# Pyrokine/LineSegmentDetector-SLAM

Hardware: AMD Instinct MI355X
Metric: Mpixels/sec LSD (grad+grow+NFA) (higher is better)
Workload: dtype f64; 1 GPU; 512 x 2048x2048 u8 occupancy maps per GPU tiled/rolled/flipped from 4 aisle-class fixtures (SURVEY 8d C4), full pipeline incl. lineIm, params 0.3/0.6/22.5/0.7/1024; images_total=512, images_rank0=512, parallelism=single GPU, rccl_gather_in_step=False, steps_in_flight=8, steps_in_flight_asked=8, region_waves_per_image=4, help_across_workgroups=False, last_steps_with_help=0, writeback_map=False

## Files before the change

include/lsd_hip.h:

```cpp
#ifndef LSD_HIP_H
#define LSD_HIP_H
#include <stddef.h>
#include <stdint.h>

#ifdef __cplusplus
extern "C" {
#endif

#define LSD_ABI_VERSION 1

enum {
    LSD_OK = 0,
    LSD_ERR_INVALID = 1,
    LSD_ERR_NO_DEVICE = 2,
    LSD_ERR_HIP = 3,
    LSD_ERR_UNSUPPORTED = 4,
    LSD_ERR_CAPACITY = 5,
    LSD_ERR_NOMEM = 6,
    LSD_ERR_INTERNAL = 7
};

typedef struct lsd_params {
    double sca;
    double sig;
// ... 213 lines not shown
                      lsd_grid_match_rec *out, lsd_grid_match_mr_stats *stats);

void lsd_scaled_size(int cols, int rows, double sca, int *w, int *h);

enum { LSD_STAGE_ALL = 0, LSD_STAGE_GAUSS = 1, LSD_STAGE_GRAD = 2, LSD_STAGE_SORT = 3, LSD_STAGE_REGION = 4 };
int lsd_set_stop_after(lsd_ctx *ctx, int stage);
int lsd_set_trace(lsd_ctx *ctx, int on);
int lsd_set_fused_front(lsd_ctx *ctx, int on);
int lsd_set_region_waves(lsd_ctx *ctx, int waves);
int lsd_set_region_help(lsd_ctx *ctx, int waves);
int lsd_set_cost_history(lsd_ctx *ctx, int on);
int lsd_debug_set_stamp_budget(lsd_ctx *ctx, unsigned grows);
int lsd_debug_set_tuning(lsd_ctx *ctx, const char *name, int value);

enum { LSD_DBG_GAUSS = 1, LSD_DBG_MAG, LSD_DBG_DEG, LSD_DBG_STATE, LSD_DBG_ORDER, LSD_DBG_ORDER_VAL,
       LSD_DBG_NB, LSD_DBG_MAXGRAD, LSD_DBG_RECS, LSD_DBG_SEEDS, LSD_DBG_NSEED, LSD_DBG_STATS };
int lsd_debug_fetch(lsd_ctx *ctx, int image, int what, void *out, size_t bytes);

int lsd_debug_eval_math(lsd_ctx *ctx, int fn, const double *a, const double *b, double *out0, double *out1, size_t n);

int lsd_debug_lines(lsd_ctx *ctx, const double *recs, int n, int cols, int rows, lsd_line *lines_out, uint8_t *line_im);

int lsd_debug_calibrate(lsd_ctx *ctx, size_t bytes);

int lsd_last_timings(lsd_ctx *ctx, float ms_out[6]);

#ifdef __cplusplus
}
#endif
#endif
```

linesegmentdetector-slam_amd/__init__.py:

```python
import ctypes as C
import os

import numpy as np

_HERE = os.path.dirname(os.path.abspath(__file__))
LIB_PATH = os.path.join(_HERE, "liblsdhip.so")

LSD_OK, LSD_ERR_INVALID, LSD_ERR_NO_DEVICE, LSD_ERR_HIP, LSD_ERR_UNSUPPORTED, LSD_ERR_CAPACITY, LSD_ERR_NOMEM, LSD_ERR_INTERNAL = range(8)
LSD_FLAG_WRITEBACK_MAP = 1
STAGE_ALL, STAGE_GAUSS, STAGE_GRAD, STAGE_SORT, STAGE_REGION = range(5)
(DBG_GAUSS, DBG_MAG, DBG_DEG, DBG_STATE, DBG_ORDER, DBG_ORDER_VAL, DBG_NB, DBG_MAXGRAD, DBG_RECS, DBG_SEEDS,
 DBG_NSEED, DBG_STATS) = range(1, 13)

lsd_sca, lsd_sig, lsd_angThre, lsd_denThre, pseBin = 0.3, 0.6, 22.5, 0.7, 1024
z_occ_max_dis = 1.0
HOST_MAX_LINES_DEFAULT = 8192
rdp_leastPoint, rdp_threLine, rdp_leastDist = 3, 0.08, 0.5


class lsd_params(C.Structure):
    _fields_ = [("sca", C.c_double), ("sig", C.c_double), ("angThre", C.c_double), ("denThre", C.c_double),
                ("pseBin", C.c_int)]


class lsd_line(C.Structure):
    _fields_ = [(n, C.c_double) for n in ("k", "b", "dx", "dy", "x1", "y1", "x2", "y2", "len")] + [("orient", C.c_int)]

# ... 664 lines not shown
            d = dict(zip(("grow_calls", "grown_px", "nfa_calls", "rrr_calls", "rrr_passes", "rrr_sentinel_drops",
                          "rrr_oob_reads", "cycles_refill", "cycles_total", "cycles_grow", "cycles_rect",
                          "cycles_nfa", "cycles_mark", "small_bails", "wait_noslot", "seeds", "exact_angle_evals",
                          "tile_fetches", "batches", "cycles_tiles", "spec_redos", "spec_discards", "cycles_wait", "small_steps",
                          "refill_rounds", "cycles_eval", "cycles_sums", "cycles_refine", "cycles_small", "cycles_select", "cycles_commit",
                          "wait_noseed", "requeued_ahead", "cycles_eval_at_cursor", "depth_end", "nfa_min_abs_enc", "nfa_min_gap_enc", "help_exports", "help_evals", "near_ties",
                          "wd_commit", "wd_next", "wd_nseeds", "wd_state", "wd_nbig", "wd_lock", "wd_pend", "wd_wave"),
                         [int(x) for x in v]))
            d["set_answers"], d["sets_founded"] = int(v[41]), int(v[42])
            d["cycles_nfa_count"], d["nfa_tail_iters"] = int(v[43]), int(v[44])
            d["nfa_bracket_misses"] = int(v[40])
            for k in ("nfa_min_abs", "nfa_min_gap"):
                enc = d.pop(k + "_enc")
                d[k] = float("inf") if enc == 0 else float(np.array([0x7ff0000000000000 - enc], np.uint64).view(np.float64)[0])
            return d
        if what == DBG_SEEDS:
            ns = self.fetch(image, DBG_NSEED, shape_wh)
            return get(what, SEED_DTYPE, ns)
        raise ValueError(what)

    def eval_math(self, fn, a, b=None):
        a = np.ascontiguousarray(a, np.float64)
        b = None if b is None else np.ascontiguousarray(b, np.float64)
        o0, o1 = np.zeros_like(a), np.zeros_like(a)
        self._chk(self.L.lsd_debug_eval_math(self.h, fn, a.ctypes.data, None if b is None else b.ctypes.data,
                                             o0.ctypes.data, o1.ctypes.data, a.size))
        return o0, o1

    def debug_lines(self, recs, rows, cols, want_lineim=True):
        r = np.ascontiguousarray(recs, np.float64).reshape(-1, 4)
# ... 1036 lines not shown
```

linesegmentdetector-slam_amd/csrc/k_front.hip:

```cpp
#include "lsd_internal.h"
#include "k_front_lds.h"
#include "k1_stage.h"
#include "grad_px.h"

namespace lsdhip {

constexpr int TW = kK1TileW, TH = kK1TileH, NT = 256;
constexpr int GW = kFrontGW, GH = kFrontGH;
constexpr int HS = 17, TAPR = 8;
constexpr int PPT = TW * TH / NT;
static_assert(TW == 32 && TW * TH % NT == 0, "a thread keeps its column and walks down the tile NT / TW rows at a time");

__global__ __launch_bounds__(NT, 4) void k_front(const uint8_t* __restrict__ in, double* __restrict__ mag, double* __restrict__ deg,
                                                 double2* __restrict__ sc, uint32_t* __restrict__ pw, unsigned long long* __restrict__ maxbits,
                                                 int32_t* __restrict__ ties, const double* __restrict__ taps_g, const int* __restrict__ centre_of,
                                                 int W, int H, int w, int h, double gradThre, int IWp, unsigned strip_bytes, unsigned gx,
                                                 unsigned gy, unsigned tiles, uint8_t* __restrict__ clr) {
    extern __shared__ __align__(16) unsigned char smem[];
    double* aux = reinterpret_cast<double*>(smem);
    double* taps = reinterpret_cast<double*>(smem + strip_bytes);
    uint8_t* tile = reinterpret_cast<uint8_t*>(taps + 3 * HS);
    double* Gt = reinterpret_cast<double*>(tile);
    int* l_cnt = reinterpret_cast<int*>(Gt + GW * GH);
    unsigned long long* l_max = reinterpret_cast<unsigned long long*>(l_cnt + 2);
    double2* l_g = reinterpret_cast<double2*>(smem);
    uint32_t* l_px = reinterpret_cast<uint32_t*>(l_g + kFrontList);

    const int tid = threadIdx.x;
    const unsigned per = (tiles + 7u) >> 3;
    const unsigned t = (blockIdx.x & 7u) * per + (blockIdx.x >> 3);
    if (t >= tiles) return;
    const unsigned bx = t % gx, tq = t / gx, by = tq % gy;
// ... 13 lines not shown
    }
    const int Xf = max(X0 - 1, 0), Yf = max(Y0 - 1, 0);
    const int Xl = min(X0 + TW - 1, w - 1), Yl = min(Y0 + TH - 1, h - 1);
    const int c0 = centre_of[Xf] - TAPR, c1 = centre_of[Xl] + TAPR;
    const int r0 = centre_of[Yf] - TAPR, r1 = centre_of[Yl] + TAPR;
    const int IH = r1 - r0 + 1;

    for (int i = tid; i < 3 * HS; i += NT) taps[i] = taps_g[i];

    const int a0 = c0 - (((c0 % 4) + 4) % 4);
    const uint32_t wany = stage_window(src, tile, W, H, r0, r1, a0, c1, IWp, tid, 0u);

    const int X = tid & (TW - 1), Yt = tid / TW;
    const int gX = X0 + X;
    if (!__syncthreads_or((int)(wany != 0u))) {
        if (gX < w) {
            #pragma unroll
            for (int k = 0; k < PPT; k++) {
                const int gY = Y0 + Yt + k * (NT / TW);
                if (gY >= h) break;
                const GradPx px = grad_pixel(0.0, 0.0, 0.0, 0.0, gX >= 1 && gY >= 1, gradThre);
                const size_t p = base + (size_t)gY * w + gX;
                mag[p] = px.m;
                if (!px.heavy && px.u == 0) sc[p] = make_double2(0.0, 1.0);
                deg[p] = px.d;
                pw[p] = pack_pw(px.d, px.u);
            }
        }
        return;
    }
// ... 75 lines not shown
    }
    {
        unsigned long long bits = (unsigned long long)__double_as_longlong(mx);
        for (int off = 32; off >= 1; off >>= 1) {
            const unsigned long long o = __shfl_xor(bits, off);
            bits = o > bits ? o : bits;
        }
        if (lane == 0) l_max[wave] = bits;
    }
    __syncthreads();
    if (tid == 0) {
        unsigned long long bits = l_max[0];
        #pragma unroll
        for (int i = 1; i < NT / 64; i++) bits = l_max[i] > bits ? l_max[i] : bits;
        if (bits != 0ull) atomicMax(&maxbits[img], bits);
    }

    const int cnt = *l_cnt;
    for (int i = tid; i < cnt; i += NT) {
        const uint32_t e = l_px[i];
        const double2 gr = l_g[i];
        const double d = grad_angle(gr.x, gr.y, &ties[img]);
        l_g[i] = make_double2(d, 0.0);
        if (e & 1u) {
            const int lt = (int)(e >> 1);
            sc[base + (size_t)(Y0 + lt / TW) * w + (X0 + lt % TW)] = grad_sincos(d);
        }
    }
    __syncthreads();

// ... 9 lines not shown
            }
        }
    }
}

bool front_fits(const Geom& g, size_t max_lds) {
    if (2 * g.tapR + 1 != HS) return false;
    const size_t need = k_front_lds(g.sca, g.tapR).bytes;
    return need <= 64 * 1024 && need <= max_lds;
}

void launch_front(const Geom& g, const Buffers& b, int n, uint8_t* clr, hipStream_t s) {
    const KFrontLds L = k_front_lds(g.sca, g.tapR);
    const unsigned gx = (g.w + TW - 1) / TW, gy = (g.h + TH - 1) / TH, tiles = gx * gy * (unsigned)n;
    hipLaunchKernelGGL(k_front, dim3(((tiles + 7u) >> 3) * 8u), dim3(NT), L.bytes, s, b.in, b.mag, b.deg, b.sc, b.pw, b.maxbits, b.ties, b.taps,
                       b.centres, g.W, g.H, g.w, g.h, g.gradThre, L.IWp, (unsigned)L.strip, gx, gy, tiles, clr);
}

}
```

linesegmentdetector-slam_amd/csrc/k_sort.hip:

```cpp
#include "lsd_internal.h"

namespace lsdhip {

constexpr int SNT = 1024, SWAVES = SNT / 64;

__device__ __forceinline__ int bin_of(double m, double zoom, int pseBin) {
    int v = cvt_x86(floor(m * zoom));
    if (v > pseBin) v = pseBin;
    return (int)(uint16_t)v;
}

__global__ __launch_bounds__(SNT) void k_sort(const double* __restrict__ mag,
                                              const unsigned long long* __restrict__ maxbits,
                                              uint32_t* __restrict__ ord,
                                              int32_t* __restrict__ nb, uint32_t* __restrict__ kept_px, uint32_t* __restrict__ kept_v32,
                                              int npx, int pseBin) {
    extern __shared__ uint32_t hist[];
    uint32_t* wsum = hist + SWAVES * pseBin;
    const size_t img = blockIdx.x;
    const double* m = mag + img * (size_t)npx;
    uint32_t* o = ord + img * (size_t)npx;
    uint32_t* kp = kept_px + img * (size_t)npx;
    uint16_t* kv = reinterpret_cast<uint16_t*>(kept_v32 + img * (size_t)npx);
    const int tid = threadIdx.x, wave = tid >> 6, lane = tid & 63;

    const double maxGrad = __longlong_as_double((long long)maxbits[img]);
    if (!(maxGrad > 0)) {
        if (tid == 0) nb[img] = 0;
        return;
    }
    const double zoom = 1.0 * pseBin / maxGrad;
    const int segLen = ((npx + SNT - 1) / SNT) * 64;
    const int beg = min(wave * segLen, npx), end = min(beg + segLen, npx);

    for (int i = tid; i < SWAVES * pseBin; i += SNT) hist[i] = 0;
    __syncthreads();

    uint32_t* myh = hist + wave * pseBin;
    const unsigned long long lt = (1ull << lane) - 1ull;
    constexpr int UN = 4;
    int cnt = 0;
    for (int base = beg; base < end; base += 64 * UN) {
        double mv[UN];
        #pragma unroll
        for (int j = 0; j < UN; j++) {
            const int p = base + 64 * j + lane;
            mv[j] = p < end ? m[p] : 0.0;
        }
        #pragma unroll
        for (int j = 0; j < UN; j++) {
            const int v = bin_of(mv[j], zoom, pseBin);
            const unsigned long long km = __ballot(v != 0);
            if (v != 0) {
                atomicAdd(&myh[pseBin - v], 1u);
                const int k2 = beg + cnt + __builtin_popcountll(km & lt);
                kp[k2] = (uint32_t)(base + 64 * j + lane);
                kv[k2] = (uint16_t)v;
            }
            cnt += __builtin_popcountll(km);
        }
    }
    __syncthreads();

    {
        uint32_t tot = 0;
        if (tid < pseBin)
            for (int s = 0; s < SWAVES; s++) tot += hist[s * pseBin + tid];
        uint32_t inc = tot;
        for (int off = 1; off < 64; off <<= 1) {
            uint32_t t = __shfl_up(inc, off);
            if (lane >= off) inc += t;
        }
        if (lane == 63) wsum[wave] = inc;
        __syncthreads();
// ... 29 lines not shown
            for (int bit = 0; bit < nbits; bit++) {
                const bool one = ((b >> bit) & 1) != 0;
                const unsigned long long mk = __ballot(one);
                peers &= one ? mk : ~mk;
            }
            const uint32_t start = myh[b];
            if (act) {
                const uint32_t r = start + (uint32_t)__builtin_popcountll(peers & lt);
                o[r] = pv[j];
                if (((peers >> lane) >> 1) == 0ull) myh[b] = start + (uint32_t)__builtin_popcountll(peers);
            }
        }
    }
}

__global__ __launch_bounds__(256) void k_order(const int32_t* __restrict__ nb, const long long* __restrict__ hist, uint32_t* __restrict__ order, int n, int npx) {
    __shared__ uint32_t cnt[256];
    __shared__ uint32_t start[256];
    __shared__ unsigned long long hmax;
    const int tid = threadIdx.x;
    cnt[tid] = 0;
    if (tid == 0) hmax = 1ull;
    __syncthreads();
    if (hist) {
        unsigned long long m = 0;
        for (int i = tid; i < n; i += 256) m = max(m, (unsigned long long)max(hist[(size_t)i * kStatWords + kStatTotalWord], 0ll));
        atomicMax(&hmax, m);
        __syncthreads();
    }
    const unsigned long long hm = hmax;
    auto key = [&](int i) {
        if (hist) return 255 - (int)(((unsigned long long)max(hist[(size_t)i * kStatWords + kStatTotalWord], 0ll) * 255ull) / hm);
        return 255 - (int)min(255ll, (long long)nb[i] * 2048 / (npx + 1));
    };
    for (int i = tid; i < n; i += 256) atomicAdd(&cnt[key(i)], 1u);
    __syncthreads();
    if (tid == 0) {
        uint32_t run = 0;
        for (int k2 = 0; k2 < 256; k2++) { start[k2] = run; run += cnt[k2]; }
    }
    __syncthreads();
    uint32_t pos = start[tid];
    for (int i = 0; i < n; i++)
        if (key(i) == tid) order[pos++] = (uint32_t)i;
}

void launch_order(const Buffers& b, int n, int npx, const long long* hist, hipStream_t s) {
    hipLaunchKernelGGL(k_order, dim3(1), dim3(256), 0, s, b.nb, hist, b.order, n, npx);
}

__global__ __launch_bounds__(256) void k_ordv(const double* __restrict__ mag, const unsigned long long* __restrict__ maxbits, const uint32_t* __restrict__ ord,
                                              uint16_t* __restrict__ out, int count, int pseBin) {
    const int i = blockIdx.x * 256 + threadIdx.x;
    const double maxGrad = __longlong_as_double((long long)maxbits[0]);
    if (i < count && maxGrad > 0) out[i] = (uint16_t)bin_of(mag[ord[i]], 1.0 * pseBin / maxGrad, pseBin);
}
void launch_ordv(const double* mag, const unsigned long long* maxbits, const uint32_t* ord, uint16_t* out, int count, int pseBin, hipStream_t s) {
    if (count > 0) hipLaunchKernelGGL(k_ordv, dim3((count + 255) / 256), dim3(256), 0, s, mag, maxbits, ord, out, count, pseBin);
}

void launch_sort(const Geom& g, const Buffers& b, int n, hipStream_t s) {
    const size_t lds = ((size_t)SWAVES * g.pseBin + SWAVES) * sizeof(uint32_t);
    (void)hipFuncSetAttribute(reinterpret_cast<const void*>(k_sort), hipFuncAttributeMaxDynamicSharedMemorySize,
                              (int)lds);
    hipLaunchKernelGGL(k_sort, dim3(n), dim3(SNT), lds, s, b.mag, b.maxbits, b.ord, b.nb, b.seedidx, b.seedpos, g.npx, g.pseBin);
}

}
```

linesegmentdetector-slam_amd/csrc/lsd_ctx.hip:

```cpp
#include <math.h>
#include <stddef.h>
#include <stdio.h>
#include <stdlib.h>
#include <string.h>

#include <algorithm>
#include <mutex>
#include <string>
#include <vector>

#include "lsd_devbuf.h"
#include "lsd_internal.h"
#include "k1_lds.h"
#include "k_rdp_lds.h"

using namespace lsdhip;

struct Workspace {
    size_t cap_gpx = 0;
    size_t cap_n = 0, cap_npx = 0, cap_ws = 0;
    int cap_max_lines = 0;
    DevBuf<double> gauss, mag, deg, recs, recs_scaled;
    DevBuf<double2> sc;
    DevBuf<uint32_t> order;
    DevBuf<uint32_t> sets;
    DevBuf<uint32_t> pw, epochmap, ord, spill, gcopy, stamps, seedidx, seedpos, tepoch;
    uint32_t run_id = 0;
    DevBuf<uint32_t> slist;
    DevBuf<double> pend;
    DevBuf<float4> wmeta;
    DevBuf<int> rnum;
    DevBuf<uint32_t> xq;
    DevBuf<unsigned long long> maxbits;
    DevBuf<int32_t> nb, nseed;
    DevBuf<long long> stats;
    DevBuf<SeedRec> seeds;
    int32_t* ties() const { return reinterpret_cast<int32_t*>(maxbits.get() + cap_n); }
};

struct lsd_ctx {
    int device = 0;
    int num_cus = 256;
    size_t max_lds = 0;
    uint32_t id_budget = 0xFFFF0u;
    int tun_soft = 0, tun_claim = 0, tun_feed = 3, tun_big = 0;
    int tun_help = -1;
    int tun_gate = 12000;
    int tun_share = 0;
    int pool_max_images = 4;
    int tun_early = 0, tun_wb = 10, tun_up = 32, tun_down = 96, tun_requeue = 1, tun_xpoll = 20000, tun_linger = 1000000, tun_stop = 0;
    int region_waves_mode = 0;
    bool prefer4 = false;
// ... 39 lines not shown
    hipEvent_t ga_ev = nullptr;
    bool ga_ev_valid = false;
    int stop_after = 0;
    int tun_groups = -1;
    DevBuf<int> pcount;
    bool trace = false;
    bool fused_front = true;
    int scan_cap = kRdpShortMaxLen;
    bool rdp_long_ready = false;
    int host_max_lines = 8192;
    Geom geom{};
    int last_n = 0;
    int last_max_lines = 0;
    int32_t* last_counts = nullptr;
    bool last_fused = false, last_remapped = false;
    const uint8_t* last_in = nullptr;
    DevBuf<double> dbg_gauss;
    hipEvent_t ev[7]{};
    bool ev_valid = false;
    hipEvent_t ev_done = nullptr;
    bool done_valid = false;
    hipStream_t done_stream = nullptr;
};

constexpr size_t kPinBytes = 32u << 20;

#define HIPCHK(ctx, call)                                                                         \
    do {                                                                                          \
        hipError_t e_ = (call);                                                                   \
        if (e_ != hipSuccess) {                                                                   \
// ... 135 lines not shown
    const long long p = free_slots < want ? free_slots : want;
    return p > 0 ? (int)p : 0;
}
static int pool_for(const lsd_ctx* c, int n) { return pool_for(c, n, c->tun_help); }
static int pool_reserve_for(const lsd_ctx* c, int n) {
    const int now = c->tun_help < 0 ? 24 : c->tun_help;
    return pool_for(c, n, now > 24 ? now : 24);
}

static bool use_front(const lsd_ctx* c, const Geom& g) {
    return c->fused_front && !c->trace && (c->stop_after == 0 || c->stop_after >= LSD_STAGE_GRAD) && front_fits(g, c->max_lds);
}
static size_t gauss_elems(const lsd_ctx* c, const Geom& g) { return use_front(c, g) ? 0 : (size_t)g.gp * g.h; }

static size_t tm_words(size_t npx) { return npx / 16 + 4 * 8200; }

static int ensure_workspace_impl(lsd_ctx* c, size_t n, size_t npx, size_t gpx, int max_lines, bool trace) {
    Workspace& w = c->ws;
    const size_t need_ws = (n + (size_t)pool_reserve_for(c, (int)n)) * (size_t)waves_for(c, (int)n);
    const bool grow_main = n > w.cap_n || npx > w.cap_npx || gpx > w.cap_gpx || need_ws > w.cap_ws;
    if (grow_main) {
        const size_t nn = n > w.cap_n ? n : w.cap_n, pp = npx > w.cap_npx ? npx : w.cap_npx;
        const size_t gg = gpx > w.cap_gpx ? gpx : w.cap_gpx;
        const size_t ws = need_ws > w.cap_ws ? need_ws : w.cap_ws;
        HIPCHK(c, hipDeviceSynchronize());
        const size_t tot = nn * pp;
        HIPCHK(c, w.gauss.resize(nn * gg)); HIPCHK(c, w.mag.resize(tot)); HIPCHK(c, w.deg.resize(tot));
        HIPCHK(c, w.sc.resize(tot));
        HIPCHK(c, w.pw.resize(tot)); HIPCHK(c, w.epochmap.resize(tot)); HIPCHK(c, w.ord.resize(tot));
        HIPCHK(c, w.spill.resize(ws * pp)); HIPCHK(c, w.gcopy.resize(ws * pp)); HIPCHK(c, w.wmeta.resize(ws * (size_t)c->mcap));
        HIPCHK(c, w.stamps.resize(ws * tm_words(pp))); HIPCHK(c, w.seedidx.resize(tot)); HIPCHK(c, w.seedpos.resize(tot)); HIPCHK(c, w.tepoch.resize(nn * (pp / 16 + 4096)));
        HIPCHK(c, hipMemset(w.stamps.get(), 0, ws * tm_words(pp) * sizeof(uint32_t)));
        HIPCHK(c, hipMemset(w.epochmap.get(), 0, tot * sizeof(uint32_t)));
        w.run_id = 0;
        const size_t gs = ws * (size_t)region_slots();
        HIPCHK(c, w.slist.resize(gs * (size_t)c->gcap));
        HIPCHK(c, w.pend.resize(gs * 24));
        HIPCHK(c, w.order.resize(nn));
        HIPCHK(c, w.sets.resize(nn * 256));
        HIPCHK(c, w.xq.resize(nn * (size_t)(kXStride + 1) + kXHdr));
        HIPCHK(c, w.maxbits.resize(nn + (nn + 1) / 2)); HIPCHK(c, w.nb.resize(nn)); HIPCHK(c, w.nseed.resize(nn));
        HIPCHK(c, w.stats.resize(nn * kStatWords)); HIPCHK(c, w.rnum.resize(nn * (size_t)region_ring() * 2));
        HIPCHK(c, w.seeds.resize(0));
        if (nn != w.cap_n) { w.cap_max_lines = 0; }
        w.cap_n = nn; w.cap_npx = pp; w.cap_gpx = gg; w.cap_ws = ws;
    }
    if (max_lines > w.cap_max_lines) {
        HIPCHK(c, hipDeviceSynchronize());
        HIPCHK(c, w.recs.resize(w.cap_n * (size_t)max_lines * 12));
        HIPCHK(c, w.recs_scaled.resize(w.cap_n * (size_t)max_lines * 4));
        w.cap_max_lines = max_lines;
    }
    if (trace && !w.seeds.get()) {
        HIPCHK(c, hipDeviceSynchronize());
        HIPCHK(c, w.seeds.resize(w.cap_n * w.cap_npx));
    }
// ... 237 lines not shown
    b.max_lines = max_lines;
    {
        const int nw = waves_for(c, n);
        b.tun_soft = c->tun_soft > 0 ? c->tun_soft : 48 * nw;
        b.tun_claim = c->tun_claim > 0 ? c->tun_claim : 192 * nw;
        b.tun_feed = c->tun_feed;
        b.tun_big = c->tun_big > 0 ? c->tun_big : 3;
        b.tun_help = c->tun_help >= 0 ? c->tun_help : 0;
        b.tun_early = c->tun_early; b.tun_wb = c->tun_wb; b.tun_gate = c->tun_gate; b.tun_share = c->tun_share; b.tun_up = c->tun_up; b.tun_down = c->tun_down; b.tun_requeue = c->tun_requeue;
        b.tun_xpoll = c->tun_xpoll; b.tun_linger = c->tun_linger; b.tun_stop = c->tun_stop;
        b.xq = (b.tun_help > 0 && !c->trace) ? w.xq.get() : nullptr;
        b.npool = b.xq ? pool_for(c, n) : 0;
    }
    b.taps = c->d_taps.get(); b.centres = c->d_centres.get(); b.lgamma = c->d_lgamma.get(); b.lg_count = (int)c->d_lgamma.capacity(); b.ptab = c->d_ptab.get();
    b.seeds = c->trace ? w.seeds.get() : nullptr; b.nseed = w.nseed.get(); b.stats = w.stats.get();

    HIPCHK(c, hipMemsetAsync(w.maxbits.get(), 0, sizeof(unsigned long long) * w.cap_n + sizeof(int32_t) * (size_t)n, s));
    const bool full_region = c->stop_after == 0 || c->stop_after >= LSD_STAGE_REGION;
    if (!full_region) HIPCHK(c, hipMemsetAsync(d_counts, 0, sizeof(int32_t) * n, s));
    if (c->stop_after != 0 && c->stop_after < LSD_STAGE_SORT) HIPCHK(c, hipMemsetAsync(w.nb.get(), 0, sizeof(int32_t) * (size_t)n, s));

    HIPCHK(c, hipEventRecord(c->ev[0], s));
    const bool fused_clear = d_line_ims && (((size_t)cols * rows) & 15) == 0 && (reinterpret_cast<uintptr_t>(d_line_ims) & 15) == 0;
    if (d_line_ims && !fused_clear) launch_clear(d_line_ims, (size_t)n * cols * rows, c->num_cus, s);
    if (fused) launch_front(g, b, n, fused_clear ? d_line_ims : nullptr, s);
    else launch_gauss(g, b, n, fused_clear ? d_line_ims : nullptr, false, s);
    if (b.in_rw) launch_remap_writeback(g, b, n, s);
    HIPCHK(c, hipEventRecord(c->ev[1], s));
    if (!fused && (c->stop_after == 0 || c->stop_after >= LSD_STAGE_GRAD)) launch_gradient(g, b, n, s);
    HIPCHK(c, hipEventRecord(c->ev[2], s));
    if (c->stop_after == 0 || c->stop_after >= LSD_STAGE_SORT) { launch_sort(g, b, n, s); launch_order(b, n, g.npx, (c->cost_history && c->hist_n == n && !c->trace) ? w.stats.get() : nullptr, s); }
    HIPCHK(c, hipEventRecord(c->ev[3], s));
    hipStream_t sr = s;
    if (c->stop_after == 0 || c->stop_after >= LSD_STAGE_REGION) {
        if (++w.run_id >= 1023u) {
            HIPCHK(c, hipMemsetAsync(w.stamps.get(), 0, w.cap_ws * tm_words(w.cap_npx) * sizeof(uint32_t), sr));
            HIPCHK(c, hipMemsetAsync(w.epochmap.get(), 0, w.cap_n * w.cap_npx * sizeof(uint32_t), sr));
            w.run_id = 1;
        }
        if (b.xq) HIPCHK(c, hipMemsetAsync(b.xq, 0, sizeof(uint32_t) * ((size_t)n * (kXStride + 1) + kXHdr), sr));
        const bool wide = waves_for(c, n) == 8;
        int grid = n;
        const int groups = c->tun_groups >= 0 ? c->tun_groups : c->num_cus;
        if (wide && groups > 0 && groups < n && !b.xq && !c->trace) {
            if (!c->pcount.get()) HIPCHK(c, c->pcount.resize(16));
            HIPCHK(c, hipMemsetAsync(c->pcount.get(), 0, sizeof(int), sr));
// ... 1 lines not shown
            grid = groups;
        }
        if (wide) launch_region_w8(g, b, grid, w.run_id << 20, sr);
        else launch_region_w4(g, b, grid, w.run_id << 20, sr);
    }
    HIPCHK(c, hipEventRecord(c->ev[4], s));
    if (c->stop_after == 0) launch_lines(g, b, n, s);
    HIPCHK(c, hipEventRecord(c->ev[5], s));
    HIPCHK(c, hipEventRecord(c->ev_done, s));
    c->done_valid = true; c->done_stream = s;
    HIPCHK(c, hipGetLastError());
    c->ev_valid = true;
    c->hist_n = (c->stop_after == 0 || c->stop_after >= LSD_STAGE_REGION) ? n : 0;
    c->geom = g; c->last_n = n; c->last_max_lines = max_lines; c->last_counts = d_counts; c->last_stream = s;
    c->last_fused = fused; c->last_in = d_maps; c->last_remapped = b.in_rw != nullptr;
    return LSD_OK;
}

int lsd_synchronize(lsd_ctx* c) {
    if (!c) return LSD_ERR_INVALID;
    HIPCHK(c, hipSetDevice(c->device));
    HIPCHK(c, hipStreamSynchronize(c->last_stream));
    return LSD_OK;
}

int lsd_last_timings(lsd_ctx* c, float ms[6]) {
    if (!c || !ms || !c->ev_valid) return LSD_ERR_INVALID;
    HIPCHK(c, hipSetDevice(c->device));
    HIPCHK(c, hipEventSynchronize(c->ev[5]));
    for (int i = 0; i < 5; i++) HIPCHK(c, hipEventElapsedTime(&ms[i], c->ev[i], c->ev[i + 1]));
    HIPCHK(c, hipEventElapsedTime(&ms[5], c->ev[0], c->ev[5]));
    if (c->last_fused) ms[1] = 0.0f;
    return LSD_OK;
}

static int h2d_staged(lsd_ctx* c, void* dst, const void* src, size_t bytes, hipStream_t s) {
    size_t off = 0;
    for (int k = 0; off < bytes; k++) {
        const int b = k & 1;
        const size_t len = bytes - off < kPinBytes ? bytes - off : kPinBytes;
        if (c->pin_used[b]) HIPCHK(c, hipEventSynchronize(c->pin_ev[b]));
        memcpy(c->pin[b], (const uint8_t*)src + off, len);
        HIPCHK(c, hipMemcpyAsync((uint8_t*)dst + off, c->pin[b], len, hipMemcpyHostToDevice, s));
        HIPCHK(c, hipEventRecord(c->pin_ev[b], s));
        c->pin_used[b] = true;
        off += len;
    }
// ... 173 lines not shown
                HIPCHK(c, tmp.resize((size_t)(nbv > 0 ? nbv : 1)));
                launch_ordv(w.mag.get() + off, w.maxbits.get() + image, w.ord.get() + off, tmp.get(), nbv, c->geom.pseBin, c->last_stream);
                HIPCHK(c, hipStreamSynchronize(c->last_stream));
                if (nbv > 0) HIPCHK(c, hipMemcpy(out, tmp.get(), (size_t)nbv * 2, hipMemcpyDeviceToHost));
                return LSD_OK;
            }
            break;
        case LSD_DBG_NB: src = w.nb.get() + image; need = 4; break;
        case LSD_DBG_MAXGRAD: src = w.maxbits.get() + image; need = 8; break;
        case LSD_DBG_RECS:
            HIPCHK(c, hipMemcpy(&cnt, c->last_counts + image, 4, hipMemcpyDeviceToHost));
            if (cnt > c->last_max_lines) cnt = c->last_max_lines;
            src = w.recs.get() + (size_t)image * c->last_max_lines * 12; need = (size_t)cnt * 12 * 8;
            break;
        case LSD_DBG_NSEED: src = w.nseed.get() + image; need = 4; break;
        case LSD_DBG_SEEDS:
            if (!w.seeds.get()) return LSD_ERR_INVALID;
            HIPCHK(c, hipMemcpy(&nseed, w.nseed.get() + image, 4, hipMemcpyDeviceToHost));
            src = w.seeds.get() + off; need = (size_t)nseed * sizeof(SeedRec);
            break;
        case LSD_DBG_STATS:
            src = w.stats.get() + (size_t)image * kStatWords; need = 8 * kStatWords;
            if (bytes > need) { const size_t all = (size_t)(c->last_n - image) * need; need = bytes < all ? bytes / need * need : all; }
            break;
        default: return LSD_ERR_INVALID;
    }
    if (bytes < need) return LSD_ERR_INVALID;
    if (need) HIPCHK(c, hipMemcpy(out, src, need, hipMemcpyDeviceToHost));
    if (what == LSD_DBG_STATE) {
        uint32_t* o = static_cast<uint32_t*>(out);
// ... 883 lines not shown
```

linesegmentdetector-slam_amd/csrc/lsd_internal.h:

```cpp
#pragma once
#include <hip/hip_runtime.h>
#include <stdint.h>
#include "../../include/lsd_hip.h"

namespace lsdhip {

constexpr double kPi = 3.14159265358979323846;
constexpr int kCentreCount = 32768;
constexpr int kMaxTapRadius = 40;
constexpr int kLgTable = 16384;
constexpr int kLgTableMax = 1 << 23;
constexpr int kStatWords = 48;
constexpr int kStatTiesWord = 39;
constexpr int kStatTotalWord = 8;
constexpr int kPTable = 16;
constexpr int kXStride = 768, kXReq = 64, kXHdr = 16;

struct Geom {
    int W, H;
    int w, h;
    int npx;
    int gp;
    double sca;
    int tapR;
// ... 55 lines not shown
    double* pend;
    double* recs;
    double* recs_scaled;
    int32_t* counts;
    lsd_line* lines;
    uint8_t* line_im;
    int max_lines;
    const double* taps;
    const int* centres;
    const double* lgamma;
    int lg_count;
    const double* ptab;
    void* seeds;
    int32_t* nseed;
    long long* stats;
};

struct SeedRec {
    int order_idx, x, y, num, outcome, final_num;
    double logNFA;
};

hipError_t prepare_gauss(const Geom& g);
void launch_gauss(const Geom& g, const Buffers& b, int n, uint8_t* clr, bool remapped, hipStream_t s);
bool front_fits(const Geom& g, size_t max_lds);
void launch_front(const Geom& g, const Buffers& b, int n, uint8_t* clr, hipStream_t s);
void launch_remap_writeback(const Geom& g, const Buffers& b, int n, hipStream_t s);
void launch_gradient(const Geom& g, const Buffers& b, int n, hipStream_t s);
void launch_sort(const Geom& g, const Buffers& b, int n, hipStream_t s);
void launch_ordv(const double* mag, const unsigned long long* maxbits, const uint32_t* ord, uint16_t* out, int count, int pseBin, hipStream_t s);
void launch_order(const Buffers& b, int n, int npx, const long long* hist, hipStream_t s);
void launch_region_w4(const Geom& g, const Buffers& b, int n, uint32_t id_base, hipStream_t s);
void launch_region_w8(const Geom& g, const Buffers& b, int n, uint32_t id_base, hipStream_t s);
int region_slots();
int region_waves();
int region_ring();
void launch_calib(double* buf, size_t n, hipStream_t s);
void launch_match(const double* map_cache, int cols, int rows, const lsd_line* map_lines, const lsd_line* scan_lines,
                  const double* pts, int n_points, double lidx, double lidy, double lastx, double lasty, const int* pairs,
                  int n_pairs, double zmax, double max_esti_dist, double* out, hipStream_t s);
void launch_occ_to_map(const uint8_t* in, uint8_t* out, size_t n, hipStream_t s);
void launch_mapcache_spread(const uint8_t* maps, double* out, unsigned long long* claim, uint32_t* fr_a, uint32_t* fr_b, int* ctl,
                            int* cnt, int n, int G, int W, int H, double res, double zmax, int cell_radius, hipStream_t s);
void launch_mapcache(const uint8_t* maps, double* out, unsigned long long* claim, uint32_t* fr_a, uint32_t* fr_b, int n,
                     int W, int H, double res, double zmax, int cell_radius, hipStream_t s);
void launch_lines(const Geom& g, const Buffers& b, int n, hipStream_t s);
// ... 68 lines not shown
```

Baseline: 69340 Mpix/s.

## Skip empty front tiles in sort and fold image ordering into sort kernel

```diff
diff --git a/include/lsd_hip.h b/include/lsd_hip.h
--- a/include/lsd_hip.h
+++ b/include/lsd_hip.h
@@ -251,7 +251,7 @@
 int lsd_debug_set_tuning(lsd_ctx *ctx, const char *name, int value);
 
 enum { LSD_DBG_GAUSS = 1, LSD_DBG_MAG, LSD_DBG_DEG, LSD_DBG_STATE, LSD_DBG_ORDER, LSD_DBG_ORDER_VAL,
-       LSD_DBG_NB, LSD_DBG_MAXGRAD, LSD_DBG_RECS, LSD_DBG_SEEDS, LSD_DBG_NSEED, LSD_DBG_STATS };
+       LSD_DBG_NB, LSD_DBG_MAXGRAD, LSD_DBG_RECS, LSD_DBG_SEEDS, LSD_DBG_NSEED, LSD_DBG_STATS, LSD_DBG_IMAGE_ORDER };
 int lsd_debug_fetch(lsd_ctx *ctx, int image, int what, void *out, size_t bytes);
 
 int lsd_debug_eval_math(lsd_ctx *ctx, int fn, const double *a, const double *b, double *out0, double *out1, size_t n);
diff --git a/linesegmentdetector-slam_amd/__init__.py b/linesegmentdetector-slam_amd/__init__.py
--- a/linesegmentdetector-slam_amd/__init__.py
+++ b/linesegmentdetector-slam_amd/__init__.py
@@ -10,7 +10,7 @@
 LSD_FLAG_WRITEBACK_MAP = 1
 STAGE_ALL, STAGE_GAUSS, STAGE_GRAD, STAGE_SORT, STAGE_REGION = range(5)
 (DBG_GAUSS, DBG_MAG, DBG_DEG, DBG_STATE, DBG_ORDER, DBG_ORDER_VAL, DBG_NB, DBG_MAXGRAD, DBG_RECS, DBG_SEEDS,
- DBG_NSEED, DBG_STATS) = range(1, 13)
+ DBG_NSEED, DBG_STATS, DBG_IMAGE_ORDER) = range(1, 14)
 
 lsd_sca, lsd_sig, lsd_angThre, lsd_denThre, pseBin = 0.3, 0.6, 22.5, 0.7, 1024
 z_occ_max_dis = 1.0
@@ -705,6 +705,8 @@
                 enc = d.pop(k + "_enc")
                 d[k] = float("inf") if enc == 0 else float(np.array([0x7ff0000000000000 - enc], np.uint64).view(np.float64)[0])
             return d
+        if what == DBG_IMAGE_ORDER:
+            return get(what, np.uint32, image + 1)
         if what == DBG_SEEDS:
             ns = self.fetch(image, DBG_NSEED, shape_wh)
             return get(what, SEED_DTYPE, ns)
diff --git a/linesegmentdetector-slam_amd/csrc/k_front.hip b/linesegmentdetector-slam_amd/csrc/k_front.hip
--- a/linesegmentdetector-slam_amd/csrc/k_front.hip
+++ b/linesegmentdetector-slam_amd/csrc/k_front.hip
@@ -15,7 +15,7 @@
                                                  double2* __restrict__ sc, uint32_t* __restrict__ pw, unsigned long long* __restrict__ maxbits,
                                                  int32_t* __restrict__ ties, const double* __restrict__ taps_g, const int* __restrict__ centre_of,
                                                  int W, int H, int w, int h, double gradThre, int IWp, unsigned strip_bytes, unsigned gx,
-                                                 unsigned gy, unsigned tiles, uint8_t* __restrict__ clr) {
+                                                 unsigned gy, unsigned tiles, uint8_t* __restrict__ clr, uint32_t* __restrict__ tilemax) {
     extern __shared__ __align__(16) unsigned char smem[];
     double* aux = reinterpret_cast<double*>(smem);
     double* taps = reinterpret_cast<double*>(smem + strip_bytes);
@@ -59,6 +59,7 @@
     const int X = tid & (TW - 1), Yt = tid / TW;
     const int gX = X0 + X;
     if (!__syncthreads_or((int)(wany != 0u))) {
+        if (tid == 0) tilemax[t] = 0u;
         if (gX < w) {
             #pragma unroll
             for (int k = 0; k < PPT; k++) {
@@ -164,6 +165,7 @@
         #pragma unroll
         for (int i = 1; i < NT / 64; i++) bits = l_max[i] > bits ? l_max[i] : bits;
         if (bits != 0ull) atomicMax(&maxbits[img], bits);
+        tilemax[t] = bits != 0ull ? 1u : 0u;
     }
 
     const int cnt = *l_cnt;
@@ -203,7 +205,7 @@
     const KFrontLds L = k_front_lds(g.sca, g.tapR);
     const unsigned gx = (g.w + TW - 1) / TW, gy = (g.h + TH - 1) / TH, tiles = gx * gy * (unsigned)n;
     hipLaunchKernelGGL(k_front, dim3(((tiles + 7u) >> 3) * 8u), dim3(NT), L.bytes, s, b.in, b.mag, b.deg, b.sc, b.pw, b.maxbits, b.ties, b.taps,
-                       b.centres, g.W, g.H, g.w, g.h, g.gradThre, L.IWp, (unsigned)L.strip, gx, gy, tiles, clr);
-}
-
-}
+                       b.centres, g.W, g.H, g.w, g.h, g.gradThre, L.IWp, (unsigned)L.strip, gx, gy, tiles, clr, b.tilemax);
+}
+
+}
diff --git a/linesegmentdetector-slam_amd/csrc/k_sort.hip b/linesegmentdetector-slam_amd/csrc/k_sort.hip
--- a/linesegmentdetector-slam_amd/csrc/k_sort.hip
+++ b/linesegmentdetector-slam_amd/csrc/k_sort.hip
@@ -1,4 +1,5 @@
 #include "lsd_internal.h"
+#include "k1_lds.h"
 
 namespace lsdhip {
 
@@ -10,54 +11,135 @@
     return (int)(uint16_t)v;
 }
 
-__global__ __launch_bounds__(SNT) void k_sort(const double* __restrict__ mag,
-                                              const unsigned long long* __restrict__ maxbits,
-                                              uint32_t* __restrict__ ord,
-                                              int32_t* __restrict__ nb, uint32_t* __restrict__ kept_px, uint32_t* __restrict__ kept_v32,
-                                              int npx, int pseBin) {
-    extern __shared__ uint32_t hist[];
+constexpr size_t kSkipLdsMax = 8192;
+static int skip_words(int npx) {
+    const int nchunks = (npx + 63) >> 6;
+    return ((nchunks + 63) >> 6) * 2 + 2;
+}
+static int tile_words(int tpi) { return ((tpi + 63) >> 6) * 2; }
+
+template <bool SPARSE>
+__device__ __forceinline__ void sort_image(uint32_t* hist, const double* __restrict__ mag, const unsigned long long* __restrict__ maxbits,
+                                           uint32_t* __restrict__ ord, int32_t* __restrict__ nb, uint32_t* __restrict__ kept_px,
+                                           uint32_t* __restrict__ kept_v32, int npx, int pseBin, const uint32_t* __restrict__ tilemax, int w,
+                                           int gx, int tpi, int ntw, int nskw) {
     uint32_t* wsum = hist + SWAVES * pseBin;
+    uint32_t* tb = wsum + SWAVES;
+    uint32_t* sk = tb + ntw;
     const size_t img = blockIdx.x;
     const double* m = mag + img * (size_t)npx;
     uint32_t* o = ord + img * (size_t)npx;
     uint32_t* kp = kept_px + img * (size_t)npx;
     uint16_t* kv = reinterpret_cast<uint16_t*>(kept_v32 + img * (size_t)npx);
-    const int tid = threadIdx.x, wave = tid >> 6, lane = tid & 63;
+    const int tid = threadIdx.x, lane = tid & 63;
+    const int wave = SPARSE ? __builtin_amdgcn_readfirstlane(tid >> 6) : tid >> 6;
 
     const double maxGrad = __longlong_as_double((long long)maxbits[img]);
     if (!(maxGrad > 0)) {
-        if (tid == 0) nb[img] = 0;
+        if (tid == SNT - 1) nb[img] = 0;
         return;
     }
     const double zoom = 1.0 * pseBin / maxGrad;
     const int segLen = ((npx + SNT - 1) / SNT) * 64;
     const int beg = min(wave * segLen, npx), end = min(beg + segLen, npx);
 
+    if (SPARSE) {
+        const uint32_t* tm = tilemax + img * (size_t)tpi;
+        for (int t0 = wave * 64; t0 < ntw * 32; t0 += SNT) {
+            const int t = t0 + lane;
+            const unsigned long long bal = __ballot(t < tpi && tm[t] != 0u);
+            if (lane == 0) { tb[t0 >> 5] = (uint32_t)bal; tb[(t0 >> 5) + 1] = (uint32_t)(bal >> 32); }
+        }
+    }
     for (int i = tid; i < SWAVES * pseBin; i += SNT) hist[i] = 0;
+    if (SPARSE) {
+        __syncthreads();
+        const int nchunks = (npx + 63) >> 6;
+        for (int c0 = wave * 64; c0 < nskw * 32; c0 += SNT) {
+            const int c = c0 + lane;
+            bool live = false;
+            if (c < nchunks) {
+                int p = c << 6;
+                const int q = min(p + 63, npx - 1);
+                int y = p / w, x = p - y * w;
+                while (p <= q) {
+                    const int xe = min(w - 1, x + (q - p));
+                    const int row = (y / kK1TileH) * gx;
+                    for (int t = row + x / kK1TileW; t <= row + xe / kK1TileW; t++) live |= ((tb[t >> 5] >> (t & 31)) & 1u) != 0u;
+                    p += xe - x + 1; y++; x = 0;
+                }
+            }
+            const unsigned long long bal = __ballot(live);
+            if (lane == 0) { sk[c0 >> 5] = (uint32_t)bal; sk[(c0 >> 5) + 1] = (uint32_t)(bal >> 32); }
+        }
+    }
     __syncthreads();
 
     uint32_t* myh = hist + wave * pseBin;
     const unsigned long long lt = (1ull << lane) - 1ull;
     constexpr int UN = 4;
     int cnt = 0;
-    for (int base = beg; base < end; base += 64 * UN) {
-        double mv[UN];
-        #pragma unroll
-        for (int j = 0; j < UN; j++) {
-            const int p = base + 64 * j + lane;
-            mv[j] = p < end ? m[p] : 0.0;
-        }
-        #pragma unroll
-        for (int j = 0; j < UN; j++) {
-            const int v = bin_of(mv[j], zoom, pseBin);
-            const unsigned long long km = __ballot(v != 0);
-            if (v != 0) {
-                atomicAdd(&myh[pseBin - v], 1u);
-                const int k2 = beg + cnt + __builtin_popcountll(km & lt);
-                kp[k2] = (uint32_t)(base + 64 * j + lane);
-                kv[k2] = (uint16_t)v;
-            }
-            cnt += __builtin_popcountll(km);
+    if (SPARSE) {
+        const int cb = beg >> 6, ce = beg < end ? (end + 63) >> 6 : cb;
+        int wb = cb - 32;
+        uint32_t win = 0u;
+        auto next_live = [&]() -> int {
+            while (win == 0u) {
+                wb += 32;
+                if (wb >= ce) return -1;
+                const unsigned long long two = (unsigned long long)sk[wb >> 5] | ((unsigned long long)sk[(wb >> 5) + 1] << 32);
+                win = __builtin_amdgcn_readfirstlane((uint32_t)(two >> (wb & 31)));
+                if (ce - wb < 32) win &= (1u << (ce - wb)) - 1u;
+            }
+            const int k = __builtin_ctz(win);
+            win &= win - 1u;
+            return wb + k;
+        };
+        for (;;) {
+            int c[UN];
+            #pragma unroll
+            for (int j = 0; j < UN; j++) c[j] = next_live();
+            if (c[0] < 0) break;
+            double mv[UN];
+            #pragma unroll
+            for (int j = 0; j < UN; j++) {
+                const int p = c[j] * 64 + lane;
+                mv[j] = (c[j] >= 0 && p < end) ? m[p] : 0.0;
+            }
+            #pragma unroll
+            for (int j = 0; j < UN; j++) {
+                if (c[j] < 0) break;
+                const int v = bin_of(mv[j], zoom, pseBin);
+                const unsigned long long km = __ballot(v != 0);
+                if (v != 0) {
+                    atomicAdd(&myh[pseBin - v], 1u);
+                    const int k2 = beg + cnt + __builtin_popcountll(km & lt);
+                    kp[k2] = (uint32_t)(c[j] * 64 + lane);
+                    kv[k2] = (uint16_t)v;
+                }
+                cnt += __builtin_popcountll(km);
+            }
+        }
+    } else {
+        for (int base = beg; base < end; base += 64 * UN) {
+            double mv[UN];
+            #pragma unroll
+            for (int j = 0; j < UN; j++) {
+                const int p = base + 64 * j + lane;
+                mv[j] = p < end ? m[p] : 0.0;
+            }
+            #pragma unroll
+            for (int j = 0; j < UN; j++) {
+                const int v = bin_of(mv[j], zoom, pseBin);
+                const unsigned long long km = __ballot(v != 0);
+                if (v != 0) {
+                    atomicAdd(&myh[pseBin - v], 1u);
+                    const int k2 = beg + cnt + __builtin_popcountll(km & lt);
+                    kp[k2] = (uint32_t)(base + 64 * j + lane);
+                    kv[k2] = (uint16_t)v;
+                }
+                cnt += __builtin_popcountll(km);
+            }
         }
     }
     __syncthreads();
@@ -117,39 +199,80 @@
     }
 }
 
-__global__ __launch_bounds__(256) void k_order(const int32_t* __restrict__ nb, const long long* __restrict__ hist, uint32_t* __restrict__ order, int n, int npx) {
-    __shared__ uint32_t cnt[256];
-    __shared__ uint32_t start[256];
-    __shared__ unsigned long long hmax;
+__device__ __forceinline__ void order_images(const int32_t* nb, const long long* __restrict__ hist, uint32_t* __restrict__ order, int n, int npx,
+                                             uint32_t* cnt, uint32_t* start, unsigned long long* hmax, uint8_t* keys, int cap) {
     const int tid = threadIdx.x;
-    cnt[tid] = 0;
-    if (tid == 0) hmax = 1ull;
+    const bool on = tid < 256;
+    if (on) cnt[tid] = 0;
+    if (tid == 0) *hmax = 1ull;
     __syncthreads();
     if (hist) {
-        unsigned long long m = 0;
-        for (int i = tid; i < n; i += 256) m = max(m, (unsigned long long)max(hist[(size_t)i * kStatWords + kStatTotalWord], 0ll));
-        atomicMax(&hmax, m);
+        if (on) {
+            unsigned long long m = 0;
+            for (int i = tid; i < n; i += 256) m = max(m, (unsigned long long)max(hist[(size_t)i * kStatWords + kStatTotalWord], 0ll));
+            atomicMax(hmax, m);
+        }
         __syncthreads();
     }
-    const unsigned long long hm = hmax;
+    const unsigned long long hm = *hmax;
     auto key = [&](int i) {
         if (hist) return 255 - (int)(((unsigned long long)max(hist[(size_t)i * kStatWords + kStatTotalWord], 0ll) * 255ull) / hm);
-        return 255 - (int)min(255ll, (long long)nb[i] * 2048 / (npx + 1));
+        const int32_t nbi = __hip_atomic_load(nb + i, __ATOMIC_RELAXED, __HIP_MEMORY_SCOPE_AGENT);
+        return 255 - (int)min(255ll, (long long)nbi * 2048 / (npx + 1));
     };
-    for (int i = tid; i < n; i += 256) atomicAdd(&cnt[key(i)], 1u);
+    const bool cached = n <= cap;
+    if (on)
+        for (int i = tid; i < n; i += 256) {
+            const int k = key(i);
+            atomicAdd(&cnt[k], 1u);
+            if (cached) keys[i] = (uint8_t)k;
+        }
     __syncthreads();
     if (tid == 0) {
         uint32_t run = 0;
         for (int k2 = 0; k2 < 256; k2++) { start[k2] = run; run += cnt[k2]; }
     }
     __syncthreads();
-    uint32_t pos = start[tid];
-    for (int i = 0; i < n; i++)
-        if (key(i) == tid) order[pos++] = (uint32_t)i;
-}
-
-void launch_order(const Buffers& b, int n, int npx, const long long* hist, hipStream_t s) {
-    hipLaunchKernelGGL(k_order, dim3(1), dim3(256), 0, s, b.nb, hist, b.order, n, npx);
+    if (on) {
+        uint32_t pos = start[tid];
+        if (cached) {
+            const uint32_t* k4 = reinterpret_cast<const uint32_t*>(keys);
+            for (int i = 0; i < n; i += 4) {
+                const uint32_t q = k4[i >> 2];
+                #pragma unroll
+                for (int j = 0; j < 4; j++)
+                    if (i + j < n && ((q >> (8 * j)) & 255u) == (uint32_t)tid) order[pos++] = (uint32_t)(i + j);
+            }
+        } else {
+            for (int i = 0; i < n; i++)
+                if (key(i) == tid) order[pos++] = (uint32_t)i;
+        }
+    }
+}
+
+template <bool SPARSE>
+__global__ __launch_bounds__(SNT) void k_sort(const double* __restrict__ mag,
+                                              const unsigned long long* __restrict__ maxbits,
+                                              uint32_t* __restrict__ ord,
+                                              int32_t* nb, uint32_t* __restrict__ kept_px, uint32_t* __restrict__ kept_v32,
+                                              int npx, int pseBin, const uint32_t* __restrict__ tilemax, int w, int gx, int tpi, int ntw, int nskw,
+                                              const long long* __restrict__ cost, uint32_t* __restrict__ order, uint32_t* ticket, int n) {
+    extern __shared__ uint32_t hist[];
+    __shared__ uint32_t o_cnt[256], o_start[256];
+    __shared__ unsigned long long o_hmax;
+    __shared__ uint32_t o_last;
+    sort_image<SPARSE>(hist, mag, maxbits, ord, nb, kept_px, kept_v32, npx, pseBin, tilemax, w, gx, tpi, ntw, nskw);
+
+    if (threadIdx.x == SNT - 1) {
+        __builtin_amdgcn_fence(__ATOMIC_RELEASE, "agent");
+        const uint32_t tk = __hip_atomic_fetch_add(ticket, 1u, __ATOMIC_RELAXED, __HIP_MEMORY_SCOPE_AGENT);
+        const bool last = tk == (uint32_t)(n - 1);
+        if (last) __builtin_amdgcn_fence(__ATOMIC_ACQUIRE, "agent");
+        o_last = last ? 1u : 0u;
+    }
+    __syncthreads();
+    if (o_last == 0u) return;
+    order_images(nb, cost, order, n, npx, o_cnt, o_start, &o_hmax, reinterpret_cast<uint8_t*>(hist), SWAVES * pseBin * (int)sizeof(uint32_t));
 }
 
 __global__ __launch_bounds__(256) void k_ordv(const double* __restrict__ mag, const unsigned long long* __restrict__ maxbits, const uint32_t* __restrict__ ord,
@@ -162,11 +285,20 @@
     if (count > 0) hipLaunchKernelGGL(k_ordv, dim3((count + 255) / 256), dim3(256), 0, s, mag, maxbits, ord, out, count, pseBin);
 }
 
-void launch_sort(const Geom& g, const Buffers& b, int n, hipStream_t s) {
-    const size_t lds = ((size_t)SWAVES * g.pseBin + SWAVES) * sizeof(uint32_t);
-    (void)hipFuncSetAttribute(reinterpret_cast<const void*>(k_sort), hipFuncAttributeMaxDynamicSharedMemorySize,
-                              (int)lds);
-    hipLaunchKernelGGL(k_sort, dim3(n), dim3(SNT), lds, s, b.mag, b.maxbits, b.ord, b.nb, b.seedidx, b.seedpos, g.npx, g.pseBin);
-}
-
-}
+void launch_sort(const Geom& g, const Buffers& b, int n, const uint32_t* tilemax, const long long* hist, hipStream_t s) {
+    const int gx = (g.w + kK1TileW - 1) / kK1TileW, gy = (g.h + kK1TileH - 1) / kK1TileH;
+    const int nskw = skip_words(g.npx), ntw = tile_words(gx * gy);
+    const bool sparse = tilemax != nullptr && (size_t)(nskw + ntw) * sizeof(uint32_t) <= kSkipLdsMax;
+    const size_t lds = ((size_t)SWAVES * g.pseBin + SWAVES + (sparse ? ntw + nskw : 0)) * sizeof(uint32_t);
+    if (sparse) {
+        (void)hipFuncSetAttribute(reinterpret_cast<const void*>(k_sort<true>), hipFuncAttributeMaxDynamicSharedMemorySize, (int)lds);
+        hipLaunchKernelGGL(k_sort<true>, dim3(n), dim3(SNT), lds, s, b.mag, b.maxbits, b.ord, b.nb, b.seedidx, b.seedpos, g.npx, g.pseBin, tilemax,
+                           g.w, gx, gx * gy, ntw, nskw, hist, b.order, b.ticket, n);
+    } else {
+        (void)hipFuncSetAttribute(reinterpret_cast<const void*>(k_sort<false>), hipFuncAttributeMaxDynamicSharedMemorySize, (int)lds);
+        hipLaunchKernelGGL(k_sort<false>, dim3(n), dim3(SNT), lds, s, b.mag, b.maxbits, b.ord, b.nb, b.seedidx, b.seedpos, g.npx, g.pseBin,
+                           (const uint32_t*)nullptr, g.w, gx, gx * gy, 0, 0, hist, b.order, b.ticket, n);
+    }
+}
+
+}
diff --git a/linesegmentdetector-slam_amd/csrc/lsd_ctx.hip b/linesegmentdetector-slam_amd/csrc/lsd_ctx.hip
--- a/linesegmentdetector-slam_amd/csrc/lsd_ctx.hip
+++ b/linesegmentdetector-slam_amd/csrc/lsd_ctx.hip
@@ -25,6 +25,7 @@
     DevBuf<uint32_t> order;
     DevBuf<uint32_t> sets;
     DevBuf<uint32_t> pw, epochmap, ord, spill, gcopy, stamps, seedidx, seedpos, tepoch;
+    DevBuf<uint32_t> tilemax;
     uint32_t run_id = 0;
     DevBuf<uint32_t> slist;
     DevBuf<double> pend;
@@ -36,6 +37,7 @@
     DevBuf<long long> stats;
     DevBuf<SeedRec> seeds;
     int32_t* ties() const { return reinterpret_cast<int32_t*>(maxbits.get() + cap_n); }
+    uint32_t* ticket(int n) const { return reinterpret_cast<uint32_t*>(ties() + n); }
 };
 
 struct lsd_ctx {
@@ -105,6 +107,7 @@
     int last_max_lines = 0;
     int32_t* last_counts = nullptr;
     bool last_fused = false, last_remapped = false;
+    bool last_sorted = false;
     const uint8_t* last_in = nullptr;
     DevBuf<double> dbg_gauss;
     hipEvent_t ev[7]{};
@@ -270,6 +273,7 @@
 static size_t gauss_elems(const lsd_ctx* c, const Geom& g) { return use_front(c, g) ? 0 : (size_t)g.gp * g.h; }
 
 static size_t tm_words(size_t npx) { return npx / 16 + 4 * 8200; }
+static size_t front_tiles(size_t npx) { return npx / ((size_t)kK1TileW * kK1TileH) + 32768 / kK1TileW + 32768 / kK1TileH + 1; }
 
 static int ensure_workspace_impl(lsd_ctx* c, size_t n, size_t npx, size_t gpx, int max_lines, bool trace) {
     Workspace& w = c->ws;
@@ -286,6 +290,7 @@
         HIPCHK(c, w.pw.resize(tot)); HIPCHK(c, w.epochmap.resize(tot)); HIPCHK(c, w.ord.resize(tot));
         HIPCHK(c, w.spill.resize(ws * pp)); HIPCHK(c, w.gcopy.resize(ws * pp)); HIPCHK(c, w.wmeta.resize(ws * (size_t)c->mcap));
         HIPCHK(c, w.stamps.resize(ws * tm_words(pp))); HIPCHK(c, w.seedidx.resize(tot)); HIPCHK(c, w.seedpos.resize(tot)); HIPCHK(c, w.tepoch.resize(nn * (pp / 16 + 4096)));
+        HIPCHK(c, w.tilemax.resize(nn * front_tiles(pp)));
         HIPCHK(c, hipMemset(w.stamps.get(), 0, ws * tm_words(pp) * sizeof(uint32_t)));
         HIPCHK(c, hipMemset(w.epochmap.get(), 0, tot * sizeof(uint32_t)));
         w.run_id = 0;
@@ -295,7 +300,7 @@
         HIPCHK(c, w.order.resize(nn));
         HIPCHK(c, w.sets.resize(nn * 256));
         HIPCHK(c, w.xq.resize(nn * (size_t)(kXStride + 1) + kXHdr));
-        HIPCHK(c, w.maxbits.resize(nn + (nn + 1) / 2)); HIPCHK(c, w.nb.resize(nn)); HIPCHK(c, w.nseed.resize(nn));
+        HIPCHK(c, w.maxbits.resize(nn + (nn + 2) / 2)); HIPCHK(c, w.nb.resize(nn)); HIPCHK(c, w.nseed.resize(nn));
         HIPCHK(c, w.stats.resize(nn * kStatWords)); HIPCHK(c, w.rnum.resize(nn * (size_t)region_ring() * 2));
         HIPCHK(c, w.seeds.resize(0));
         if (nn != w.cap_n) { w.cap_max_lines = 0; }
@@ -563,8 +568,9 @@
     }
     b.taps = c->d_taps.get(); b.centres = c->d_centres.get(); b.lgamma = c->d_lgamma.get(); b.lg_count = (int)c->d_lgamma.capacity(); b.ptab = c->d_ptab.get();
     b.seeds = c->trace ? w.seeds.get() : nullptr; b.nseed = w.nseed.get(); b.stats = w.stats.get();
-
-    HIPCHK(c, hipMemsetAsync(w.maxbits.get(), 0, sizeof(unsigned long long) * w.cap_n + sizeof(int32_t) * (size_t)n, s));
+    b.tilemax = w.tilemax.get(); b.ticket = w.ticket(n);
+
+    HIPCHK(c, hipMemsetAsync(w.maxbits.get(), 0, sizeof(unsigned long long) * w.cap_n + sizeof(int32_t) * ((size_t)n + 1), s));
     const bool full_region = c->stop_after == 0 || c->stop_after >= LSD_STAGE_REGION;
     if (!full_region) HIPCHK(c, hipMemsetAsync(d_counts, 0, sizeof(int32_t) * n, s));
     if (c->stop_after != 0 && c->stop_after < LSD_STAGE_SORT) HIPCHK(c, hipMemsetAsync(w.nb.get(), 0, sizeof(int32_t) * (size_t)n, s));
@@ -577,8 +583,9 @@
     if (b.in_rw) launch_remap_writeback(g, b, n, s);
     HIPCHK(c, hipEventRecord(c->ev[1], s));
     if (!fused && (c->stop_after == 0 || c->stop_after >= LSD_STAGE_GRAD)) launch_gradient(g, b, n, s);
-    HIPCHK(c, hipEventRecord(c->ev[2], s));
-    if (c->stop_after == 0 || c->stop_after >= LSD_STAGE_SORT) { launch_sort(g, b, n, s); launch_order(b, n, g.npx, (c->cost_history && c->hist_n == n && !c->trace) ? w.stats.get() : nullptr, s); }
+    if (!fused) HIPCHK(c, hipEventRecord(c->ev[2], s));
+    if (c->stop_after == 0 || c->stop_after >= LSD_STAGE_SORT)
+        launch_sort(g, b, n, fused ? b.tilemax : nullptr, (c->cost_history && c->hist_n == n && !c->trace) ? w.stats.get() : nullptr, s);
     HIPCHK(c, hipEventRecord(c->ev[3], s));
     hipStream_t sr = s;
     if (c->stop_after == 0 || c->stop_after >= LSD_STAGE_REGION) {
@@ -610,6 +617,7 @@
     c->hist_n = (c->stop_after == 0 || c->stop_after >= LSD_STAGE_REGION) ? n : 0;
     c->geom = g; c->last_n = n; c->last_max_lines = max_lines; c->last_counts = d_counts; c->last_stream = s;
     c->last_fused = fused; c->last_in = d_maps; c->last_remapped = b.in_rw != nullptr;
+    c->last_sorted = c->stop_after == 0 || c->stop_after >= LSD_STAGE_SORT;
     return LSD_OK;
 }
 
@@ -624,9 +632,11 @@
     if (!c || !ms || !c->ev_valid) return LSD_ERR_INVALID;
     HIPCHK(c, hipSetDevice(c->device));
     HIPCHK(c, hipEventSynchronize(c->ev[5]));
-    for (int i = 0; i < 5; i++) HIPCHK(c, hipEventElapsedTime(&ms[i], c->ev[i], c->ev[i + 1]));
+    for (int i = 0; i < 5; i++) {
+        if (c->last_fused && i == 1) { ms[1] = 0.0f; continue; }
+        HIPCHK(c, hipEventElapsedTime(&ms[i], c->ev[c->last_fused && i == 2 ? 1 : i], c->ev[i + 1]));
+    }
     HIPCHK(c, hipEventElapsedTime(&ms[5], c->ev[0], c->ev[5]));
-    if (c->last_fused) ms[1] = 0.0f;
     return LSD_OK;
 }
 
@@ -830,6 +840,10 @@
             src = w.recs.get() + (size_t)image * c->last_max_lines * 12; need = (size_t)cnt * 12 * 8;
             break;
         case LSD_DBG_NSEED: src = w.nseed.get() + image; need = 4; break;
+        case LSD_DBG_IMAGE_ORDER:
+            if (!c->last_sorted) return LSD_ERR_INVALID;
+            src = w.order.get(); need = ((size_t)image + 1) * 4;
+            break;
         case LSD_DBG_SEEDS:
             if (!w.seeds.get()) return LSD_ERR_INVALID;
             HIPCHK(c, hipMemcpy(&nseed, w.nseed.get() + image, 4, hipMemcpyDeviceToHost));
diff --git a/linesegmentdetector-slam_amd/csrc/lsd_internal.h b/linesegmentdetector-slam_amd/csrc/lsd_internal.h
--- a/linesegmentdetector-slam_amd/csrc/lsd_internal.h
+++ b/linesegmentdetector-slam_amd/csrc/lsd_internal.h
@@ -93,6 +93,8 @@
     void* seeds;
     int32_t* nseed;
     long long* stats;
+    uint32_t* tilemax;
+    uint32_t* ticket;
 };
 
 struct SeedRec {
@@ -106,9 +108,8 @@
 void launch_front(const Geom& g, const Buffers& b, int n, uint8_t* clr, hipStream_t s);
 void launch_remap_writeback(const Geom& g, const Buffers& b, int n, hipStream_t s);
 void launch_gradient(const Geom& g, const Buffers& b, int n, hipStream_t s);
-void launch_sort(const Geom& g, const Buffers& b, int n, hipStream_t s);
+void launch_sort(const Geom& g, const Buffers& b, int n, const uint32_t* tilemax, const long long* hist, hipStream_t s);
 void launch_ordv(const double* mag, const unsigned long long* maxbits, const uint32_t* ord, uint16_t* out, int count, int pseBin, hipStream_t s);
-void launch_order(const Buffers& b, int n, int npx, const long long* hist, hipStream_t s);
 void launch_region_w4(const Geom& g, const Buffers& b, int n, uint32_t id_base, hipStream_t s);
 void launch_region_w8(const Geom& g, const Buffers& b, int n, uint32_t id_base, hipStream_t s);
 int region_slots();
```

Measured after the change: 69450 Mpix/s (median of 2 runs). About the same (+0.2%).
